# ricklisz/AnatoMask

Hardware: AMD Instinct MI355X
Metric: pretrain volumes/sec @128^3 patch mask=0.6 (higher is better)
Workload: dtype bf16; 1 GPU; STUNet-B AnatoMask step, 128^3 patch, mask_ratio 0.6, bf16 storage/MFMA + fp32 master; per_gpu_batch=16, global_batch=16, parallelism=dp1, step=teacher fwd + sampler + student fwd + loss + bwd + clip + AdamW + EMA

## Files before the change

anatomask_amd/csrc/conv_igemm.hip:

```cpp
#include <mutex>
#include <type_traits>
#include <stdlib.h>
#include "common.h"
#include "../../include/anatomask_hip.h"
#include "conv_plan.h"

using namespace amconv;

namespace {

template <typename T, int BD, int BH, int BW, int NS, int NIT, int TGS = 3, bool HR = false, bool NB = false, bool HT = false>
__global__ __launch_bounds__(256, (TGS == 2 && BD * BH * BW <= 256) ? 3 : 2) void conv_igemm_kernel(ConvArgs a) {
  constexpr int EPC = TT<T>::EPC;
  constexpr bool SPL = std::is_same<T, f32s_t>::value;
  constexpr int KC = (ROWB / 16) * EPC;
  constexpr int MV = BD * BH * BW;
  constexpr int VS = MV / 64;
  constexpr int NT = 16 * NS;
  constexpr int TG = TG_OF(NS, TGS);
  constexpr int WBUF = TG * NT * ROWB;
  constexpr int WCH = TG * NT * 4;
  constexpr int WIT = (WCH + 255) / 256;
  static_assert(MV % 64 == 0, "brick must give each wave whole 16-voxel subtiles");
  extern __shared__ __attribute__((aligned(16))) unsigned char lds[];
// ... 566 lines not shown
#ifdef AM_ABLATE
    { const char* e = getenv("AM_CV_NOLIST"); if (e && atoi(e)) listed = false; }
#endif
    if (listed) {
      a.plist = active_list; a.pbd = qblock / P.bd; a.pbh = qblock / P.bh; a.pbw = qblock / P.bw;
      a.nlive = p.n_active * a.pbd * a.pbh * a.pbw;
    }
  }
  if (p.partials && p.dtype == AM_DT_BF16) {
    const size_t tile = (size_t)P.bd * P.bh * P.bw * (P.nt_tile * 2 + 32);
    if (P.lds < tile) P.lds = tile;
  }
  if (p.nbred) {
    const size_t tiles = (size_t)P.bd * P.bh * P.bw * (P.nt_tile * 4 + 32);
    if (P.lds < tiles) P.lds = tiles;
  }
  a.nt_store = ((size_t)p.B * p.Do * p.Ho * p.Wo * p.Cout * 2 >= ((size_t)384 << 20) && !p.accumulate) || AM_DBG(a, 8);
  hipStream_t st = (hipStream_t)stream;
  if (rows) *rows = (a.plist ? a.nlive : a.B * a.nbd * a.nbh * a.nbw) * a.nclass;
  return p.dtype == AM_DT_BF16 ? dispatch<bf16_t>(P, shape, st) : p.dtype == AM_DT_F32S ? dispatch<f32s_t>(P, shape, st) : dispatch<float>(P, shape, st);
}

#define AM_STAGE_ROW(name_) {#name_, name_##_fits, name_##_serves, name_##_launch}
static const ConvStage conv_stages[] = {AM_STAGE_ROW(conv_k3t), AM_STAGE_ROW(conv_k3), AM_STAGE_ROW(conv_rw), AM_STAGE_ROW(conv_gather), AM_STAGE_ROW(conv_igemm)};

static void query_masks(ConvProblem& p, bool sparse, int in_bshift, int out_bshift, int n_active) {
  p.in_sparse = p.out_sparse = sparse; p.same_mask = p.has_list = true;
  p.in_bshift = in_bshift; p.out_bshift = out_bshift; p.n_active = n_active;
}

extern "C" int am_conv3d_partials_rows(int mode, int dtype, int ksize, int stride, int B, int Do, int Ho, int Wo, int Cin, int Cout, int out_sparse,
                                       int out_bshift, int n_active, int* rows) {
  ConvProblem p{mode, dtype, ksize, stride, B, Do, Ho, Wo, Cin, Do, Ho, Wo, Cout};
  query_masks(p, out_sparse != 0, out_bshift, out_bshift, n_active);
  *rows = 0;
  for (const ConvStage& s : conv_stages) { const int r = s.fits(p); if (r > *rows) *rows = r; }
  return 0;
}

extern "C" int am_conv3d_uses_k3(int mode, int dtype, int ksize, int stride, int B, int Di, int Hi, int Wi, int Cin, int Do, int Ho, int Wo, int Cout,
                                 int has_masks, int accumulate, int fused_epilogue, int want_partials) {
  ConvProblem p{mode, dtype, ksize, stride, B, Di, Hi, Wi, Cin, Do, Ho, Wo, Cout};
  query_masks(p, has_masks != 0, 0, 0, 0);
  p.accumulate = accumulate != 0; p.ep = fused_epilogue != 0; p.partials = want_partials != 0;
  for (const ConvStage& s : conv_stages)
    if (s.serves(p)) return s.launch == conv_k3t_launch ? 2 : s.launch == conv_k3_launch ? 1 : 0;
  return 0;
}

static ConvArgs fill_args(const ConvProblem& p, const void* x, const void* w_packed, const float* bias, void* y, float* partials, const uint8_t* in_mask,
                          int in_bshift, const uint8_t* out_mask, int out_bshift, int fd, int fh, int fw, int accumulate) {
  ConvArgs a{};
  a.x = x; a.w = w_packed; a.bias = bias; a.y = y; a.partials = partials;
  a.B = p.B; a.Di = p.Di; a.Hi = p.Hi; a.Wi = p.Wi; a.Cin = p.Cin; a.Do = p.Do; a.Ho = p.Ho; a.Wo = p.Wo; a.Cout = p.Cout;
  am_packed_dims(p.dtype, p.Cout, p.Cin, &a.Coutp, &a.Cinp);
  a.w_bytes = p.ksize * p.ksize * p.ksize * a.Coutp * a.Cinp * (p.dtype == AM_DT_BF16 ? 2 : 4);
  a.in_mask = MaskView{in_mask, fd, fh, fw, in_bshift};
  a.out_mask = MaskView{out_mask, fd, fh, fw, out_bshift};
  a.accumulate = accumulate & 1; a.stats_sum_only = (accumulate & AM_CONV_PARTIALS_SUM_ONLY) ? 1 : 0;
#ifdef AM_ABLATE
  { const char* e = getenv("AM_CV_DBG"); a.dbg = e ? atoi(e) : 0; }
#endif
  return a;
}

static int conv3d_impl(ConvProblem& p, ConvArgs& a, const int* active_list, int n_active, void* stream, int* rows) {
  if (p.Cin % 8 || p.Cout % 8) return -1;
  p.in_sparse = a.in_mask.m != nullptr; p.out_sparse = a.out_mask.m != nullptr; p.same_mask = a.in_mask.m == a.out_mask.m;
  p.in_bshift = a.in_mask.bs; p.out_bshift = a.out_mask.bs; p.fd = a.in_mask.fd; p.fh = a.in_mask.fh; p.fw = a.in_mask.fw;
  p.has_list = active_list != nullptr; p.n_active = n_active;
// ... 57 lines not shown
```

anatomask_amd/csrc/conv_k3.hip:

```cpp
#include <stdlib.h>
#include "common.h"
#include "../../include/anatomask_hip.h"
#include "conv_plan.h"

using namespace amconv;

namespace {

constexpr int KBD = 8, KBH = 4, KBW = 16;
constexpr int KED = KBD + 2, KEH = KBH + 2, KEW = KBW + 2;
constexpr int KPLANE = KEH * KEW;
constexpr int KNROW = KED * KPLANE;
constexpr int KBRICKB = KNROW * 64;
constexpr int KNPIECE = 68;
constexpr int KWSLOT = 3 * 64 * 64;
constexpr int KLDS_W = 2 * KBRICKB;
constexpr int KLDS_TAB = KLDS_W + 2 * KWSLOT;
constexpr int KLDS = KLDS_TAB + 768;
#ifndef AM_K3_MIN_UNITS
#define AM_K3_MIN_UNITS 256
#endif
constexpr int K3_MIN_UNITS = AM_K3_MIN_UNITS;

struct K3Args {
// ... 5 lines not shown
  int nt_store;
  unsigned w_bytes;
#ifdef AM_ABLATE
  int dbg;
#endif
};

#define K3_LDSP(off) ((__attribute__((address_space(3))) void*)(lds + (off)))

__device__ __forceinline__ int k3_uni(int v) { return __builtin_amdgcn_readfirstlane(v); }
template <typename P> __device__ __forceinline__ P* k3_uni_ptr(P* p) {
  const unsigned long long v = (unsigned long long)p;
  const unsigned lo = (unsigned)__builtin_amdgcn_readfirstlane((int)(unsigned)v), hi = (unsigned)__builtin_amdgcn_readfirstlane((int)(unsigned)(v >> 32));
  return (P*)(((unsigned long long)hi << 32) | lo);
}

struct Item { int u, k, c0, c1, p; };
#define IT_Q0W(it) (((it).c0 & 255) * KBW)
#define IT_Q0H(it) ((((it).c0 >> 8) & 255) * KBH)
#define IT_Q0D(it) ((((it).c0 >> 16) & 255) * KBD)
#define IT_B(it) ((it).c1 & 255)
#define IT_CO0(it) (((it).c1 >> 8) * NT)

template <int NS, bool EP, bool ST, bool CT = false, bool S1 = false>
__global__ __launch_bounds__(512, 2) void conv_k3_kernel(K3Args a) {
  static_assert(NS == 4 || NS == 2, "64- or 32-channel output tiles (NS = 2: the decoder's last conv, C -> C / 2 = 32 at STUNet-B; a wave then owns 8 accumulator tiles)");
  constexpr int VS = 4, NT = 16 * NS;
  constexpr int NCH = VS * NS / 2;
  constexpr int NRUN = CT ? 4 : 9;
  constexpr int NTR = CT ? 2 : 3;
  static_assert(!CT || (NS == 4 && !EP && !ST), "transposed conv: 64-channel tiles, plain epilogue (bias)");
  static_assert(!S1 || (ST && NS == 4 && !CT), "sum-only statistics: a variant of the statistics instantiation");
  extern __shared__ __attribute__((aligned(16))) unsigned char lds[];
  const int tid = threadIdx.x, lane = tid & 63;
  const int wave = __builtin_amdgcn_readfirstlane(tid >> 6);
  const bool isX = wave < 4;
  const int wq = wave & 3;
  const int g = lane >> 4, r16 = lane & 15;
  const int G = gridDim.x;

  const int gperm = (G % 8 == 0) ? (int)(blockIdx.x % 8) * (G / 8) + (int)(blockIdx.x / 8) : (int)blockIdx.x;
  auto decode = [&](Item& it) {
    int br = it.u / a.ny;
    const int yt = it.u - br * a.ny;
    const int bw_ = br % a.nbw; br /= a.nbw;
    const int bh_ = br % a.nbh; br /= a.nbh;
    const int bd_ = br % a.nbd;
    it.c0 = k3_uni(bw_ | (bh_ << 8) | (bd_ << 16)); it.c1 = k3_uni((br / a.nbd) | (yt << 8));
  };
  auto advance = [&](Item& it) {
    if (it.k + 1 < a.nslab) { ++it.k; return; }
    it.k = 0;
    if (CT && it.p < 7) { ++it.p; return; }
    it.p = 0; it.u += G;
    if (it.u < a.nunit) decode(it);
  };
  Item cur; cur.u = gperm; cur.k = 0; cur.p = 0;
  if (cur.u >= a.nunit) return;
  decode(cur);
  Item nxt = cur; advance(nxt);

  const __amdgpu_buffer_rsrc_t rw = __builtin_amdgcn_make_buffer_rsrc((void*)a.w, 0, (int)a.w_bytes, 0x00020000);
  constexpr unsigned OOB = 0x80000000u;
  const int wtapB = a.Coutp * a.Cinp * 2;

  const int wrow = lane >> 2;
  const unsigned wlane = (unsigned)(((((wrow >> 2) & 3) * 8 + (wrow & 3)) * a.Cinp + (((lane & 3) ^ ((wrow >> 1) & 2)) * 8)) * 2);
  const int aoff = swz(r16, g);
  int bx[3];
#pragma unroll
  for (int xw = 0; xw < 3; ++xw) bx[xw] = (wave * KPLANE + r16 + xw) * 64 + ((g ^ (((r16 + xw) >> 2) & 1) * 2) << 4);

  unsigned pl[9], pbits[2] = {0u, 0u};
#pragma unroll
  for (int k = 0; k < 9; ++k) {
    const int p = wave + 8 * k;
    const int row0 = p * 16 < KNROW - 16 ? p * 16 : KNROW - 16;
    const int rho = row0 + (lane >> 2);
    const int z = rho / KPLANE, rem = rho - z * KPLANE, yy = rem / KEW, xx = rem - yy * KEW;
    pl[k] = (unsigned)((((z * a.H + yy) * a.W + xx) * a.Cin + (((lane & 3) ^ (((xx >> 2) & 1) * 2)) * 8)) * 2);
    const unsigned code = (z == 0 ? 1u : 0u) | (z == KED - 1 ? 2u : 0u) | (yy == 0 ? 4u : 0u) | (yy == KEH - 1 ? 8u : 0u) | (xx == 0 ? 16u : 0u) | (xx == KEW - 1 ? 32u : 0u);
    pbits[k / 5] |= code << (6 * (k % 5));
  }

  auto issue_weights = [&](const Item& it, const int run, const int slot) __attribute__((always_inline)) {
    const int pd_ = (it.p >> 2) & 1, ph_ = (it.p >> 1) & 1, pw_ = it.p & 1;
    const int zd = CT ? pd_ + (run >> 1) : run / 3, xw = CT ? pw_ + (run & 1) : run - (run / 3) * 3;
    if (wq >= NS) return;
#pragma unroll
    for (int th = 0; th < NTR; ++th) {
      const int t = zd * 9 + th * 3 + xw;
      const int widx = CT ? ((3 - 2 * zd + pd_) * 4 + (3 - 2 * (ph_ + th) + ph_)) * 4 + (3 - 2 * xw + pw_) : (a.flip ? 26 - t : t);
      const unsigned so = (unsigned)(widx * wtapB + ((IT_CO0(it) + (wq >> 1) * 32 + (wq & 1) * 4) * a.Cinp + it.k * 32) * 2);
#ifdef AM_ABLATE
      if (a.dbg & 4) continue;
#endif
      __builtin_amdgcn_raw_ptr_buffer_load_lds(rw, K3_LDSP(KLDS_W + slot * KWSLOT + th * (NT * 64) + wq * 1024), 16, wlane, so, 0, 0);
    }
  };
  auto issue_pieces = [&](const Item& it, const int sbuf, const int k0, const int k1) __attribute__((always_inline)) {
    const int q0d = IT_Q0D(it), q0h = IT_Q0H(it), q0w = IT_Q0W(it);
    const unsigned m = (q0d == 0 ? 1u : 0u) | (q0d + KBD == a.D ? 2u : 0u) | (q0h == 0 ? 4u : 0u) | (q0h + KBH == a.H ? 8u : 0u) |
                       (q0w == 0 ? 16u : 0u) | (q0w + KBW == a.W ? 32u : 0u);
    const long long org = ((((long long)IT_B(it) * a.D + (q0d - 1)) * a.H + (q0h - 1)) * a.W + (q0w - 1)) * (long long)a.Cin;
    const __amdgpu_buffer_rsrc_t rx = __builtin_amdgcn_make_buffer_rsrc((void*)k3_uni_ptr(a.x + org), 0, 0x7fffff00, 0x00020000);
#pragma unroll
    for (int k = k0; k < k1; ++k) {
      const unsigned bad = pbits[k / 5] & (m << (6 * (k % 5)));
      unsigned vo = bad ? OOB : pl[k];
#ifdef AM_ABLATE
      if (a.dbg & 2) vo = OOB;
#endif
      const int p = wave + 8 * k;
      const int row0 = p * 16 < KNROW - 16 ? p * 16 : KNROW - 16;
      __builtin_amdgcn_raw_ptr_buffer_load_lds(rx, K3_LDSP(sbuf * KBRICKB + row0 * 64), 16, vo, (unsigned)(it.k * 64), 0, 0);
    }
  };

  f32x4 acc[NS][VS];
  float f1[NS / 2][4], f2[NS / 2][4];
#pragma unroll
  for (int h = 0; h < NS / 2; ++h)
#pragma unroll
    for (int r = 0; r < 4; ++r) { f1[h][r] = 0.f; f2[h][r] = 0.f; }
  const unsigned oddm = (lane & 1) ? 0xffffffffu : 0u;
#ifdef AM_ABLATE
  const bool want_stats = ST && a.partials != nullptr && !(a.dbg & 32);
#else
  const bool want_stats = ST && a.partials != nullptr;
#endif
  bf16_t* __restrict__ yg = a.y;
  const float act_slope = a.ep_act == AM_ACT_LRELU ? 0.01f : (a.ep_act == AM_ACT_RELU6 ? 0.f : 1.f);
  const float act_hi = a.ep_act == AM_ACT_RELU6 ? 6.f : __builtin_inff();
  constexpr bool fused = EP;
  typedef __attribute__((ext_vector_type(4))) __bf16 bfx4;
  typedef __attribute__((ext_vector_type(8))) __bf16 bfx8;
  typedef __attribute__((ext_vector_type(8))) float f32x8;

  auto flush_stats = [&](const int co0) __attribute__((always_inline)) {
    float* part = a.partials + ((size_t)blockIdx.x * 8 + wave) * a.Cout * 2;
#define K3_DPP_ADD(V, CTRL) V += __builtin_bit_cast(float, __builtin_amdgcn_update_dpp(0, __builtin_bit_cast(int, V), CTRL, 0xF, 0xF, true))
#pragma unroll
    for (int h = 0; h < NS / 2; ++h)
#pragma unroll
      for (int r = 0; r < 4; ++r) {
        float s1 = f1[h][r], s2 = f2[h][r];
        K3_DPP_ADD(s1, 0x4E); K3_DPP_ADD(s1, 0x124); K3_DPP_ADD(s1, 0x128);
        if constexpr (!S1) { K3_DPP_ADD(s2, 0x4E); K3_DPP_ADD(s2, 0x124); K3_DPP_ADD(s2, 0x128); }
        const int c = co0 + h * 32 + g * 8 + (r16 & 1) * 4 + r;
        if (r16 < 2) { part[c * 2] = s1; part[c * 2 + 1] = s2; }
      }
#undef K3_DPP_ADD
  };

  constexpr bool FULL = NS == 4;
  const bool lo8 = r16 < 8;
  const unsigned olane = FULL ? (unsigned)(((r16 & 7) * (CT ? 2 : 1) * a.Cout + (r16 >> 3) * 32 + g * 8) * 2)
                              : (unsigned)((r16 * (CT ? 2 : 1) * a.Cout + g * 8) * 2);
  const unsigned ohalf = (unsigned)(8 * (CT ? 2 : 1) * a.Cout * 2);
  const unsigned olane_own = (unsigned)((r16 * (CT ? 2 : 1) * a.Cout + g * 8) * 2);
  const unsigned orow = (unsigned)((CT ? 4 : 1) * a.W * a.Cout * 2);
  u32x4 pk[VS][NS / 2];
  long long pk_off = 0;
  auto finish_unit = [&](const int pc0, const int pc1, const int pcls) __attribute__((always_inline)) {
    Item it; it.c0 = pc0; it.c1 = pc1;
    const int co0 = IT_CO0(it);
    if constexpr (CT)
      pk_off = ((((long long)IT_B(it) * (2 * a.D) + (2 * (IT_Q0D(it) + wave) + ((pcls >> 2) & 1))) * (2 * a.H) + (2 * IT_Q0H(it) + ((pcls >> 1) & 1))) * (2 * a.W) +
                (2 * IT_Q0W(it) + (pcls & 1))) * (long long)a.Cout + co0;
    else
    pk_off = ((((long long)IT_B(it) * a.D + (IT_Q0D(it) + wave)) * a.H + IT_Q0H(it)) * a.W + IT_Q0W(it)) * (long long)a.Cout + co0;
    f32x4 bia[NS], esc[NS], esh[NS];
    if (a.bias) {
#pragma unroll
      for (int i = 0; i < NS; ++i) bia[i] = *(const f32x4*)(lds + KLDS_TAB + ((i >> 1) * 32 + g * 8 + (i & 1) * 4) * 4);
// ... 38 lines not shown
      }
    }
  };
  auto stats_half = [&](const int c, const int q) __attribute__((always_inline)) {
    const int j = c / (NS / 2), h = c % (NS / 2);
    const u32x4 wv = pk[j][h];
    const unsigned kw = (wv[2 + q] & oddm) | (wv[q] & ~oddm), gw = (wv[q] & oddm) | (wv[2 + q] & ~oddm);
#pragma unroll
    for (int e = 0; e < 2; ++e) {
      const int r = 2 * q + e;
      const float keep = __uint_as_float(e ? (kw & 0xffff0000u) : (kw << 16)), give = __uint_as_float(e ? (gw & 0xffff0000u) : (gw << 16));
      f1[h][r] += keep;
      f1[h][r] += __builtin_bit_cast(float, __builtin_amdgcn_update_dpp(0, __builtin_bit_cast(int, give), 0xB1, 0xF, 0xF, true));
      if constexpr (!S1) {
        f2[h][r] += keep * keep;
        const float g2 = give * give;
        f2[h][r] += __builtin_bit_cast(float, __builtin_amdgcn_update_dpp(0, __builtin_bit_cast(int, g2), 0xB1, 0xF, 0xF, true));
      }
    }
  };
#ifdef AM_K3_NO_SPREAD_STATS
  constexpr bool spread_stats = false;
#else
  const bool spread_stats = ST && !CT && NCH == 8 && a.nslab >= 2;
#endif
  auto store_chunk = [&](const int c, const bool tail) __attribute__((always_inline)) {
    const int j = c / (NS / 2), h = c % (NS / 2);
    const __amdgpu_buffer_rsrc_t ry = __builtin_amdgcn_make_buffer_rsrc((void*)k3_uni_ptr(yg + pk_off), 0, 0x7fffff00, 0x00020000);
#ifdef AM_ABLATE
    if (!(a.dbg & 1))
#endif
    {
      u32x4 sv = pk[j][h];
      unsigned so_ = (unsigned)(j * orow + h * 64);
      if constexpr (FULL) {
        const u32x4 ot = pk[j][h ^ 1];
        u32x4 rx_;
#pragma unroll
        for (int e = 0; e < 4; ++e) rx_[e] = (unsigned)__builtin_amdgcn_update_dpp(0, (int)ot[e], 0x128, 0xF, 0xF, false);
        const bool own = h == 0 ? lo8 : !lo8;
#pragma unroll
        for (int e = 0; e < 4; ++e) sv[e] = own ? sv[e] : rx_[e];
        so_ = (unsigned)(j * orow) + (h ? ohalf : 0u);
      }
      if (a.nt_store) __builtin_amdgcn_raw_buffer_store_b128(sv, ry, olane, so_, 2);
      else __builtin_amdgcn_raw_buffer_store_b128(sv, ry, olane, so_, 0);
      if (tail || FULL) asm volatile("s_nop 4" : "+v"(sv) :: "memory");
    }
    if (want_stats && (tail || !spread_stats)) { stats_half(c, 0); stats_half(c, 1); }
  };

  if (want_stats && a.ny > 1) {
    float* part = a.partials + ((size_t)blockIdx.x * 8 + wave) * a.Cout * 2;
    for (int c = lane; c < a.Cout * 2; c += 64) part[c] = 0.f;
    asm volatile("s_waitcnt vmcnt(0)" ::: "memory");
  }
  if (tid < NT) {
    const int c = IT_CO0(cur) + tid;
    ((float*)(lds + KLDS_TAB))[tid] = a.bias ? a.bias[c] : 0.f;
    ((float*)(lds + KLDS_TAB))[64 + tid] = a.ep_scale ? a.ep_scale[c] : 1.f;
    ((float*)(lds + KLDS_TAB))[128 + tid] = a.ep_scale ? a.ep_shift[c] : 0.f;
  }
  if (isX) { issue_weights(cur, 0, 0); issue_pieces(cur, 0, 0, 9); }
  else issue_pieces(cur, 0, 0, 8);
  asm volatile("s_waitcnt vmcnt(0) lgkmcnt(0)" ::: "memory");
  __builtin_amdgcn_s_barrier();

#ifdef AM_ABLATE
  unsigned tL = 0, tWL = 0, tM = 0, tWM = 0, tE = 0, t_prev = 0;
  unsigned long long rt0 = 0;
  const bool stamps = (a.dbg & 16) != 0;
#define K3_STAMP(ACC) if (stamps) { unsigned long long t_; asm volatile("s_memtime %0\n\ts_waitcnt lgkmcnt(0)" : "=s"(t_) :: "memory"); ACC += (unsigned)t_ - t_prev; t_prev = (unsigned)t_; }
  if (stamps) { unsigned long long t_; asm volatile("s_memtime %0\n\ts_waitcnt lgkmcnt(0)" : "=s"(t_) :: "memory"); t_prev = (unsigned)t_; asm volatile("s_memrealtime %0\n\ts_waitcnt lgkmcnt(0)" : "=s"(rt0) :: "memory"); }
#else
#define K3_STAMP(ACC)
#endif
  int par = 0, sb = 0;
  int pc0 = 0, pc1 = 0, pcls = 0; bool have_prev = false;
  bool spend = false;
  bool pend_stats = false;
#pragma unroll
  for (int i = 0; i < NS; ++i)
#pragma unroll
    for (int j = 0; j < VS; ++j) acc[i][j] = f32x4{0.f, 0.f, 0.f, 0.f};
  while (true) {
    spend = false;
    if (cur.k == 0 && have_prev) {
      finish_unit(pc0, pc1, pcls);
      spend = true; pend_stats = true;
      K3_STAMP(tE);
    } else if (cur.k >= 2) pend_stats = false;
    const bool has_next = nxt.u < a.nunit;
    int bxc[3];
#pragma unroll
    for (int xw = 0; xw < 3; ++xw) bxc[xw] = bx[xw] + sb * KBRICKB;
    const bool fetch_next = has_next && (!CT || a.nslab != 2 || nxt.p == 0);
    const int cpd = (cur.p >> 2) & 1, cph = (cur.p >> 1) & 1, cpw = cur.p & 1;
#pragma unroll
    for (int run = 0; run < NRUN; ++run) {
      const int zd = run / 3, xw = run % 3;
      u32x4 brow[VS + 2], af[3][NS];
      const int wbase = KLDS_W + par * KWSLOT + aoff;
      if constexpr (CT) {
        const int zq = cpd + (run >> 1), xq = cpw + (run & 1);
        const int bsel = (xq == 0 ? bxc[0] : (xq == 1 ? bxc[1] : bxc[2])) + (zq * KPLANE + cph * KEW) * 64;
#pragma unroll
        for (int r = 0; r < VS + 1; ++r) brow[r] = *(const u32x4*)(lds + bsel + r * KEW * 64);
      } else {
#pragma unroll
      for (int r = 0; r < VS + 2; ++r) brow[r] = *(const u32x4*)(lds + bxc[xw] + (zd * KPLANE + r * KEW) * 64);
      }
#pragma unroll
      for (int th = 0; th < NTR; ++th)
#pragma unroll
        for (int i = 0; i < NS; ++i) af[th][i] = *(const u32x4*)(lds + wbase + th * (NT * 64) + i * 1024);
      const int pk0 = CT ? (isX ? 3 * run : 4 * run) : (run == 0 ? 0 : (run == 1 ? 1 : run + 1));
      const int npx = CT ? (run < 3 ? 3 : 0) : (run == 1 ? 2 : (run < 8 ? 1 : 0));
      const int npy = CT ? (run < 2 ? 4 : 0) : (run == 1 ? 2 : (run < 7 ? 1 : 0));
      constexpr int SPR = CT ? 2 : 1;
      if (isX) {
        if (run < NRUN - 1) issue_weights(cur, run + 1, par ^ 1);
        else if (has_next) issue_weights(nxt, 0, par ^ 1);
        if (fetch_next && npx > 0) issue_pieces(nxt, sb ^ 1, CT ? 3 * run : pk0, (CT ? 3 * run : pk0) + npx);
        if (spend && run * SPR < NCH) {
#pragma unroll
          for (int q = 0; q < SPR; ++q) store_chunk(run * SPR + q, false);
        }
      } else {
        if (spend && run * SPR < NCH) {
#pragma unroll
          for (int q = 0; q < SPR; ++q) store_chunk(run * SPR + q, false);
        }
        if (fetch_next && npy > 0) issue_pieces(nxt, sb ^ 1, CT ? 4 * run : pk0, (CT ? 4 * run : pk0) + npy);
      }
      if (spread_stats && want_stats && pend_stats) {
        if (cur.k == 0) stats_half(run >> 1, run & 1);
        else if (cur.k == 1 && 9 + run < 16) stats_half((9 + run) >> 1, (9 + run) & 1);
      }
      K3_STAMP(tL);
      if (!isX) {
        asm volatile("s_waitcnt lgkmcnt(0)" ::: "memory");
        __builtin_amdgcn_s_barrier();
        K3_STAMP(tWL);
      }
      __builtin_amdgcn_sched_barrier(0);
      __builtin_amdgcn_s_setprio(1);
#ifdef AM_ABLATE
      if (!(a.dbg & 8))
#endif
#pragma unroll
      for (int th = 0; th < NTR; ++th)
#pragma unroll
        for (int j = 0; j < VS; ++j)
#pragma unroll
          for (int i = 0; i < NS; ++i) acc[i][j] = mma_chunk<bf16_t>(af[th][i], brow[j + th], acc[i][j]);
      __builtin_amdgcn_s_setprio(0);
      __builtin_amdgcn_sched_barrier(0);
      if (isX) {
        const int nbehind = (fetch_next ? npx : 0) + ((spend && run * SPR < NCH) ? SPR : 0);
        if (nbehind == 0) asm volatile("s_waitcnt vmcnt(0)" ::: "memory");
        else if (nbehind == 1) asm volatile("s_waitcnt vmcnt(1)" ::: "memory");
        else if (nbehind == 2) asm volatile("s_waitcnt vmcnt(2)" ::: "memory");
        else if (nbehind == 3) asm volatile("s_waitcnt vmcnt(3)" ::: "memory");
        else if (nbehind == 4) asm volatile("s_waitcnt vmcnt(4)" ::: "memory");
        else asm volatile("s_waitcnt vmcnt(5)" ::: "memory");
      } else if (run == NRUN - 2) {
        if (spend && run * SPR < NCH) { if (SPR == 2) asm volatile("s_waitcnt vmcnt(2)" ::: "memory"); else asm volatile("s_waitcnt vmcnt(1)" ::: "memory"); }
        else asm volatile("s_waitcnt vmcnt(0)" ::: "memory");
      }
      K3_STAMP(tM);
      if (isX) {
        __builtin_amdgcn_s_barrier();
        K3_STAMP(tWM);
      }
      par ^= 1;
    }
    sb ^= 1;
    if (cur.k + 1 == a.nslab) { pc0 = cur.c0; pc1 = cur.c1; pcls = cur.p; have_prev = true; }
    if (!has_next) break;
    cur = nxt; advance(nxt);
  }
  finish_unit(pc0, pc1, pcls);
#pragma unroll
  for (int c = 0; c < NCH; ++c) store_chunk(c, true);
  if (want_stats) flush_stats((pc1 >> 8) * NT);
#ifdef AM_ABLATE
  if (stamps && a.partials) {
    K3_STAMP(tE);
    unsigned long long rt1; asm volatile("s_memrealtime %0\n\ts_waitcnt lgkmcnt(0)" : "=s"(rt1) :: "memory");
    unsigned* row = (unsigned*)(a.partials + ((size_t)blockIdx.x * 8 + wave) * a.Cout * 2);
    asm volatile("s_waitcnt vmcnt(0)" ::: "memory");
    if (lane == 0) { row[0] = tL; row[1] = tWL; row[2] = tM; row[3] = tWM; row[4] = tE; row[5] = (unsigned)(rt1 - rt0); }
  }
#endif
}

}

namespace amconv {

static int k3_tiles(int Cout) { return Cout % 64 ? Cout / 32 : Cout / 64; }
// ... 23 lines not shown
#endif
  if (!conv_k3_fits(p) || p.prenorm || p.accumulate || p.nbred) return false;
  if (p.Di != p.Do || p.Hi != p.Ho || p.Wi != p.Wo) return false;
  if ((size_t)(KED + 1) * p.Hi * p.Wi * p.Cin * 2 >= 0x7fffff00ull) return false;
  if (p.ep && p.partials) return false;
  return true;
}

int conv_k3t_fits(const ConvProblem&) { return 0; }
bool conv_k3t_serves(const ConvProblem& p) {
#ifdef AM_ABLATE
  if (getenv("AM_CV_NORW")) return false;
  { const char* e_ = getenv("AM_CV_NOK3T"); if (e_ && atoi(e_)) return false; }
#endif
  if (p.mode != AM_CONVT_FWD || p.dtype != AM_DT_BF16 || p.ksize != 4 || p.stride != 2 || p.in_sparse || p.out_sparse) return false;
  if (p.prenorm || p.accumulate || p.nbred || p.partials || p.ep) return false;
  if (p.Cin % 32 || p.Cin < 64 || p.Cout % 64 || p.Di % KBD || p.Hi % KBH || p.Wi % KBW) return false;
  if (p.Do != 2 * p.Di || p.Ho != 2 * p.Hi || p.Wo != 2 * p.Wi) return false;
  if (p.B > 255 || p.Di / KBD > 255 || p.Hi / KBH > 255 || p.Wi / KBW > 255) return false;
  if ((size_t)(KED + 1) * p.Hi * p.Wi * p.Cin * 2 >= 0x7fffff00ull || (size_t)16 * p.Wo * p.Cout * 2 >= 0x7fffff00ull) return false;
  return k3_units(p.B, p.Di, p.Hi, p.Wi, p.Cout) >= K3_MIN_UNITS;
}

static void k3_fill(K3Args& a, const ConvProblem& p, const ConvArgs& c) {
  a.x = (const bf16_t*)c.x; a.w = (const bf16_t*)c.w; a.bias = c.bias; a.y = (bf16_t*)c.y; a.partials = c.partials;
  a.ep_scale = c.ep_scale; a.ep_shift = c.ep_shift; a.ep_res = (const bf16_t*)c.ep_res; a.ep_act = c.ep_act;
  a.B = c.B; a.D = c.Di; a.H = c.Hi; a.W = c.Wi; a.Cin = c.Cin; a.Cout = c.Cout; a.Cinp = c.Cinp; a.Coutp = c.Coutp;
  a.nbd = c.Di / KBD; a.nbh = c.Hi / KBH; a.nbw = c.Wi / KBW; a.ny = k3_tiles(c.Cout); a.nunit = k3_units(c.B, c.Di, c.Hi, c.Wi, c.Cout); a.nslab = c.Cinp / 32;
  a.flip = p.mode == AM_CONV_DGRAD;
  a.nt_store = (size_t)c.B * c.Do * c.Ho * c.Wo * c.Cout * 2 >= ((size_t)384 << 20);
  a.w_bytes = (unsigned)c.w_bytes;
#ifdef AM_ABLATE
  { const char* e = getenv("AM_K3_DBG"); a.dbg = e ? atoi(e) : 0; }
#endif
}

int conv_k3_launch(const ConvProblem& p, ConvArgs& c, const int*, void* stream, int* rows) {
  if (!conv_k3_serves(p)) return 0;
  const int dev = am_device();
  K3Args a;
  k3_fill(a, p, c);
  const int G = k3_grid(a.nunit, c.Cout, dev);
  auto kern = p.ep ? conv_k3_kernel<4, true, false> : (a.partials ? conv_k3_kernel<4, false, true> : conv_k3_kernel<4, false, false>);
  if (c.Cout % 64) kern = p.ep ? conv_k3_kernel<2, true, false> : (a.partials ? conv_k3_kernel<2, false, true> : conv_k3_kernel<2, false, false>);
  else if (a.partials && !p.ep && c.stats_sum_only) kern = conv_k3_kernel<4, false, true, false, true>;
  AM_HIP_STAGE((am_lds_optin<conv_k3_kernel<4, true, false>, conv_k3_kernel<4, false, true>, conv_k3_kernel<4, false, false>,
                             conv_k3_kernel<2, true, false>, conv_k3_kernel<2, false, true>, conv_k3_kernel<2, false, false>,
                             conv_k3_kernel<4, false, true, false, true>>(dev)));
  AM_LAUNCH(kern, dim3(G), dim3(512), KLDS, (hipStream_t)stream, a);
  AM_CHECK_LAUNCH_STAGE();
  if (rows) *rows = G * 8;
  return 1;
}

int conv_k3t_launch(const ConvProblem& p, ConvArgs& c, const int*, void* stream, int*) {
  if (!conv_k3t_serves(p)) return 0;
  const int dev = am_device();
  K3Args a;
  k3_fill(a, p, c);
  constexpr auto kern = conv_k3_kernel<4, false, false, true>;
  AM_HIP_STAGE(am_lds_optin<kern>(dev));
  AM_LAUNCH(kern, dim3(k3_grid(a.nunit, c.Cout, dev)), dim3(512), KLDS, (hipStream_t)stream, a);
  AM_CHECK_LAUNCH_STAGE();
  return 1;
}

}
```

anatomask_amd/csrc/conv_plan.h:

```cpp
#pragma once
#include "common.h"

namespace amconv {

struct ConvArgs {
  const void* x; const void* w; const float* bias; void* y; float* partials;
  const float* ep_scale; const float* ep_shift; const void* ep_res; int ep_act;
  const void* nb_x; const float* nb_scale; const float* nb_shift; int nb_act;
  const float* in_scale; const float* in_shift; int in_act;
  int B, Di, Hi, Wi, Cin, Do, Ho, Wo, Cout, Cinp, Coutp;
  int OS, GS, nclass, nunit;
  int ny;
  int nbd, nbh, nbw;
  int tap_begin[9];
  int upar[8];
  int taps[64];
  int mind[8], minh[8], minw[8];
  int ed[8], eh[8], ew[8];
  int mdiv_w[8], mdiv_hw[8];
  int w_bytes;
  int w_lds_off;
  MaskView in_mask, out_mask;
  int accumulate;
  int stats_sum_only;
// ... 78 lines not shown
  a.w_lds_off = (int)brick;
  P.tgs = a.nunit > 1 ? 2 : 3;
  P.lds = a.w_lds_off + 2 * TG_OF(P.nt_tile / 16, P.tgs) * P.nt_tile * ROWB;
  return 0;
}


struct ConvProblem {
  int mode, dtype, ksize, stride, B, Di, Hi, Wi, Cin, Do, Ho, Wo, Cout;
  bool in_sparse, out_sparse, same_mask, has_list;
  int in_bshift, out_bshift, n_active, fd, fh, fw;
  bool accumulate, ep, partials, sum_only;
  bool nbred, prenorm;
};

struct ConvStage {
  const char* name;
  int (*fits)(const ConvProblem&);
  bool (*serves)(const ConvProblem&);
  int (*launch)(const ConvProblem&, ConvArgs& a, const int* active_list, void* stream, int* rows);
};
#define AM_CONV_STAGE(name_) int name_##_fits(const ConvProblem&); bool name_##_serves(const ConvProblem&); \
                             int name_##_launch(const ConvProblem&, ConvArgs&, const int*, void*, int*)
AM_CONV_STAGE(conv_k3t); AM_CONV_STAGE(conv_k3);
AM_CONV_STAGE(conv_rw); AM_CONV_STAGE(conv_gather);
AM_CONV_STAGE(conv_igemm);

}
```

anatomask_amd/engine.py:

```python
from __future__ import annotations

from dataclasses import dataclass, field
from typing import Dict, List, Optional, Sequence, Tuple

import torch

from . import ops
from .ops import ACT_LRELU, ACT_NONE, ACT_RELU6, CONV_DGRAD, CONV_FWD, CONVT_DGRAD, CONVT_FWD, MaskInfo, NormStats

ENC = "sparse_encoder.sp_cnn.conv_blocks_context"
DEC = "dense_decoder.dec"


@dataclass
class Spec:
    dims: Sequence[int]
    depth: Sequence[int]
    width: int
    input_size: Tuple[int, int, int]
    in_ch: int = 1
    out_ch: int = 1
    downsample: int = 16
    n_stage: int = 5
    sync_bn: bool = False
# ... 404 lines not shown
        dr = ops.conv3d(CONV_DGRAD, dc2, pk.get(W, f"{q}.conv.3.weight", False, True), None, so, 3, 1)
        _wgrad_into(pk, G, f"{q}.conv.3.weight", CONV_FWD, t["r"], dc2, 3, 1)
        dc1 = _instance_norm_backward(dr, t["c1"], t["st1"], ACT_RELU6)
    elif t.get("head"):
        dc2 = ops.proj_norm_bwd(t["c2"], t["st2"], drec, W["dense_decoder.proj.weight"].view(-1), W[f"{q}.conv.4.weight"],
                                W[f"{q}.conv.4.bias"], G[f"{q}.conv.4.weight"], G[f"{q}.conv.4.bias"],
                                G["dense_decoder.proj.weight"].view(-1), G["dense_decoder.proj.bias"])
    else:
        dc2 = ops.norm_backward(g, None, t["c2"], t["st2"], W[f"{q}.conv.4.weight"], ACT_NONE, None, 0,
                                G[f"{q}.conv.4.weight"], G[f"{q}.conv.4.bias"])
    if not t.get("inorm"):
        so = tuple(t["r"].shape[1:4])
        fuse = ops.FUSED_NORM_BWD_REDUCE and dc2.dtype == torch.bfloat16 and t["st1"].sync_world <= 1 and dc2.shape[-1] >= 128
        dr = ops.conv3d(CONV_DGRAD, dc2, pk.get(W, f"{q}.conv.3.weight", False, True), None, so, 3, 1,
                        norm_bwd=(t["c1"], t["st1"], ACT_RELU6) if fuse else None)
        dr, red1 = dr if fuse else (dr, None)
        _wgrad_into(pk, G, f"{q}.conv.3.weight", CONV_FWD, t["r"], dc2, 3, 1)
        dc1 = ops.norm_backward(dr, None, t["c1"], t["st1"], W[f"{q}.conv.1.weight"], ACT_RELU6, None, 0,
                                G[f"{q}.conv.1.weight"], G[f"{q}.conv.1.bias"], reduced=red1)
    du, ptu = ops.conv3d(CONV_DGRAD, dc1, pk.get(W, f"{q}.conv.0.weight", False, True), None, so, 3, 1, want_partials=True, partials_sum_only=True)
    ptu.finalize(None, sum_accum=G[f"{q}.up_sample.bias"])
    _wgrad_into(pk, G, f"{q}.conv.0.weight", CONV_FWD, t["u"], dc1, 3, 1)
    si = tuple(t["xin"].shape[1:4])
    gin = ops.conv3d(CONVT_DGRAD, du, pk.get(W, f"{q}.up_sample.weight", True, True), None, si, 4, 2, want_partials=bias_sum_into is not None)
    if bias_sum_into is not None:
        gin, ptg = gin
        ptg.finalize(None, sum_accum=bias_sum_into)
    _wgrad_into(pk, G, f"{q}.up_sample.weight", CONVT_FWD, t["xin"], du, 4, 2, transposed=True)
    return gin


def decoder_backward(spec: Spec, W, G, pk: PackCache, tape: Tape, drec: torch.Tensor, after_group=None) -> List[Optional[torch.Tensor]]:
    n_dec = len(spec.dec_chs) - 1
    fused_head = bool(tape.dec[n_dec - 1].get("head"))
    g = None
    if not fused_head:
        g = ops.proj_bwd(tape.last, drec, W["dense_decoder.proj.weight"].view(-1), G["dense_decoder.proj.weight"].view(-1),
                         G["dense_decoder.proj.bias"], deterministic=pk.deterministic)
        if after_group:
            after_group("proj")
    dproj: List[Optional[torch.Tensor]] = [None] * n_dec
    for i in reversed(range(n_dec)):
        t = tape.dec[i]
        if tape.recompute:
            _, t = _dec_block(W, pk, i, t["xin"], t["nxt"], True, update_running=False, sync=spec.sync_bn, head=bool(t.get("head")),
                              inorm=spec.dec_inorm)
            tape.dec[i] = None
# ... 213 lines not shown
```

include/anatomask_hip.h:

```cpp
#ifndef ANATOMASK_HIP_H
#define ANATOMASK_HIP_H
#include <stdint.h>
#ifdef __cplusplus
extern "C" {
#endif

#define AM_DT_F32 0
#define AM_DT_BF16 1
#define AM_DT_F32S 2

#define AM_CONV_PARTIALS_SUM_ONLY 2
#define AM_CONV_FWD 0
#define AM_CONV_DGRAD 1
#define AM_CONVT_FWD 2
#define AM_CONVT_DGRAD 3

#define AM_DXREP 64
#define AM_NREP 8

#define AM_ACT_NONE 0
#define AM_ACT_LRELU 1
#define AM_ACT_RELU6 2

int am_version(void);
// ... 6 lines not shown
              const void* ep_res ,
              int ep_act ,
              const int32_t* active_list, int n_active ,
              int* partial_rows_written ,
              void* stream);
int am_conv3d_prenorm_supported(int mode, int dtype, int ksize, int stride, int B, int Do, int Ho, int Wo, int Cin, int Cout, int sparse,
                                int in_bshift, int out_bshift, int n_active);
int am_conv3d_prenorm(int mode, int dtype, int ksize, int stride, const void* x, const void* w_packed, const float* bias, void* y, int B, int Di,
                      int Hi, int Wi, int Cin, int Do, int Ho, int Wo, int Cout, const uint8_t* mask, int in_bshift, int out_bshift, int fd,
                      int fh, int fw, float* partials , const float* in_scale, const float* in_shift, int in_act,
                      const int32_t* active_list, int n_active, int* partial_rows_written , void* stream);

int am_conv3d_nbred(int mode, int dtype, int ksize, int stride, const void* x, const void* w_packed, void* y, int B, int Di,
                    int Hi, int Wi, int Cin, int Do, int Ho, int Wo, int Cout, const uint8_t* in_mask, int in_bshift,
                    const uint8_t* out_mask, int out_bshift, int fd, int fh, int fw, int accumulate, float* partials,
                    const void* nb_x, const float* nb_scale, const float* nb_shift, int nb_act,
                    int* partial_rows_written, void* stream);
int am_packed_dims(int dtype, int rows, int k, int* rows_padded, int* k_padded);
int am_conv3d_partials_rows(int mode, int dtype, int ksize, int stride, int B, int Do, int Ho, int Wo, int Cin, int Cout,
                            int out_sparse, int out_bshift ,
                            int n_active, int* rows );
int am_conv3d_uses_k3(int mode, int dtype, int ksize, int stride, int B, int Di, int Hi, int Wi, int Cin, int Do, int Ho, int Wo, int Cout,
                      int has_masks, int accumulate, int fused_epilogue, int want_partials);
int am_partials_reduce(const float* partials, int rows, int C, double* sums, float* sum_accum, void* stream);

int am_conv3d_wgrad(int mode, int dtype, int ksize, int stride, const void* x, const void* dy, float* dw_packed,
                    int B, int Dx, int Hx, int Wx, int Cx, int Dy, int Hy, int Wy, int Cy,
                    const uint8_t* x_mask, int x_bshift, const uint8_t* y_mask, int y_bshift, int fd, int fh, int fw,
                    float* det_workspace, long det_workspace_floats,
                    const int32_t* active_list, int n_active ,
                    void* gather_workspace, long gather_workspace_bytes ,
                    void* stream);
int am_conv3d_wgrad_uses_k3(int mode, int dtype, int ksize, int stride, int B, int D, int H, int W, int Cx, int Cy, int has_masks,
                            int deterministic);
int am_conv3d_wgrad_gather_bytes(int mode, int dtype, int ksize, int stride, int B, int Cx, int Cy, int y_bshift, int has_y_mask, int n_active,
                                 int fd, int fh, int fw, long* bytes );

int am_split_bf16(const float* x, void* hi, void* lo, long n, void* stream);

int am_pack_weight(int dtype, const float* src, void* dst, int R, int K, int taps, long stride_r, long stride_k, int Rp, int Kp,
                   void* stream);
typedef struct am_pack_desc {
  const float* src; void* dst; long stride_r, stride_k; int R, K, taps, Rp, Kp, first_block;
} am_pack_desc;
int am_pack_weights_batched(int dtype, const am_pack_desc* descs, int ndesc, int total_blocks, void* stream);
int am_unpack_grad(const float* src_packed, float* dst, int R, int K, int taps, long stride_r, long stride_k, int accumulate,
// ... 173 lines not shown
```

Before: 140.4 volumes/s.

## Route transposed-conv data gradient through the k3 brick kernel with parity phases

Adds a conv_k3td stage that computes the data gradient of the stride-2, 4x4x4 transposed conv on the k3 LDS-brick MFMA kernel. Each output brick iterates the 8 input parity phases as 2x2x2-tap runs over a stride-2 view of the input, accumulating all phases before the epilogue. Per-block channel statistics are reduced across waves in LDS, and the decoder requests sum-only partials. This replaces the generic igemm/gather path for these decoder backward convs, at the cost of more kernel variants and new indexing that could be wrong at edges.

```diff
diff --git a/anatomask_amd/csrc/conv_igemm.hip b/anatomask_amd/csrc/conv_igemm.hip
--- a/anatomask_amd/csrc/conv_igemm.hip
+++ b/anatomask_amd/csrc/conv_igemm.hip
@@ -1,5 +1,6 @@
 #include <mutex>
 #include <type_traits>
+#include <stdio.h>
 #include <stdlib.h>
 #include "common.h"
 #include "../../include/anatomask_hip.h"
@@ -612,7 +613,7 @@
 }
 
 #define AM_STAGE_ROW(name_) {#name_, name_##_fits, name_##_serves, name_##_launch}
-static const ConvStage conv_stages[] = {AM_STAGE_ROW(conv_k3t), AM_STAGE_ROW(conv_k3), AM_STAGE_ROW(conv_rw), AM_STAGE_ROW(conv_gather), AM_STAGE_ROW(conv_igemm)};
+static const ConvStage conv_stages[] = {AM_STAGE_ROW(conv_k3t), AM_STAGE_ROW(conv_k3td), AM_STAGE_ROW(conv_k3), AM_STAGE_ROW(conv_rw), AM_STAGE_ROW(conv_gather), AM_STAGE_ROW(conv_igemm)};
 
 static void query_masks(ConvProblem& p, bool sparse, int in_bshift, int out_bshift, int n_active) {
   p.in_sparse = p.out_sparse = sparse; p.same_mask = p.has_list = true;
@@ -636,6 +637,17 @@
   for (const ConvStage& s : conv_stages)
     if (s.serves(p)) return s.launch == conv_k3t_launch ? 2 : s.launch == conv_k3_launch ? 1 : 0;
   return 0;
+}
+
+extern "C" int am_conv3d_stage_name(int mode, int dtype, int ksize, int stride, int B, int Di, int Hi, int Wi, int Cin, int Do, int Ho, int Wo, int Cout,
+                                    int has_masks, int accumulate, int fused_epilogue, int want_partials, char* name, int cap) {
+  if (!name || cap <= 0) return -1;
+  ConvProblem p{mode, dtype, ksize, stride, B, Di, Hi, Wi, Cin, Do, Ho, Wo, Cout};
+  query_masks(p, has_masks != 0, 0, 0, 0);
+  p.accumulate = accumulate != 0; p.ep = fused_epilogue != 0; p.partials = want_partials != 0;
+  for (const ConvStage& s : conv_stages)
+    if (s.serves(p)) { snprintf(name, (size_t)cap, "%s", s.name); return 0; }
+  return -7;
 }
 
 static ConvArgs fill_args(const ConvProblem& p, const void* x, const void* w_packed, const float* bias, void* y, float* partials, const uint8_t* in_mask,
diff --git a/anatomask_amd/csrc/conv_k3.hip b/anatomask_amd/csrc/conv_k3.hip
--- a/anatomask_amd/csrc/conv_k3.hip
+++ b/anatomask_amd/csrc/conv_k3.hip
@@ -51,15 +51,17 @@
 #define IT_B(it) ((it).c1 & 255)
 #define IT_CO0(it) (((it).c1 >> 8) * NT)
 
-template <int NS, bool EP, bool ST, bool CT = false, bool S1 = false>
+template <int NS, bool EP, bool ST, bool CT = false, bool S1 = false, bool CD = false>
 __global__ __launch_bounds__(512, 2) void conv_k3_kernel(K3Args a) {
   static_assert(NS == 4 || NS == 2, "64- or 32-channel output tiles (NS = 2: the decoder's last conv, C -> C / 2 = 32 at STUNet-B; a wave then owns 8 accumulator tiles)");
   constexpr int VS = 4, NT = 16 * NS;
   constexpr int NCH = VS * NS / 2;
-  constexpr int NRUN = CT ? 4 : 9;
-  constexpr int NTR = CT ? 2 : 3;
+  constexpr bool C2 = CT || CD;
+  constexpr int NRUN = C2 ? 4 : 9;
+  constexpr int NTR = C2 ? 2 : 3;
   static_assert(!CT || (NS == 4 && !EP && !ST), "transposed conv: 64-channel tiles, plain epilogue (bias)");
   static_assert(!S1 || (ST && NS == 4 && !CT), "sum-only statistics: a variant of the statistics instantiation");
+  static_assert(!CD || (NS == 4 && !EP && !CT), "transposed conv's data gradient: 64-channel tiles, no fused store epilogue");
   extern __shared__ __attribute__((aligned(16))) unsigned char lds[];
   const int tid = threadIdx.x, lane = tid & 63;
   const int wave = __builtin_amdgcn_readfirstlane(tid >> 6);
@@ -80,7 +82,7 @@
   auto advance = [&](Item& it) {
     if (it.k + 1 < a.nslab) { ++it.k; return; }
     it.k = 0;
-    if (CT && it.p < 7) { ++it.p; return; }
+    if (C2 && it.p < 7) { ++it.p; return; }
     it.p = 0; it.u += G;
     if (it.u < a.nunit) decode(it);
   };
@@ -107,19 +109,21 @@
     const int row0 = p * 16 < KNROW - 16 ? p * 16 : KNROW - 16;
     const int rho = row0 + (lane >> 2);
     const int z = rho / KPLANE, rem = rho - z * KPLANE, yy = rem / KEW, xx = rem - yy * KEW;
-    pl[k] = (unsigned)((((z * a.H + yy) * a.W + xx) * a.Cin + (((lane & 3) ^ (((xx >> 2) & 1) * 2)) * 8)) * 2);
+    pl[k] = CD ? (unsigned)((((z * 4 * a.H + yy * 2) * 2 * a.W + xx * 2) * a.Cin + (((lane & 3) ^ (((xx >> 2) & 1) * 2)) * 8)) * 2)
+               : (unsigned)((((z * a.H + yy) * a.W + xx) * a.Cin + (((lane & 3) ^ (((xx >> 2) & 1) * 2)) * 8)) * 2);
     const unsigned code = (z == 0 ? 1u : 0u) | (z == KED - 1 ? 2u : 0u) | (yy == 0 ? 4u : 0u) | (yy == KEH - 1 ? 8u : 0u) | (xx == 0 ? 16u : 0u) | (xx == KEW - 1 ? 32u : 0u);
     pbits[k / 5] |= code << (6 * (k % 5));
   }
 
   auto issue_weights = [&](const Item& it, const int run, const int slot) __attribute__((always_inline)) {
     const int pd_ = (it.p >> 2) & 1, ph_ = (it.p >> 1) & 1, pw_ = it.p & 1;
-    const int zd = CT ? pd_ + (run >> 1) : run / 3, xw = CT ? pw_ + (run & 1) : run - (run / 3) * 3;
+    const int zd = C2 ? pd_ + (run >> 1) : run / 3, xw = C2 ? pw_ + (run & 1) : run - (run / 3) * 3;
     if (wq >= NS) return;
 #pragma unroll
     for (int th = 0; th < NTR; ++th) {
       const int t = zd * 9 + th * 3 + xw;
-      const int widx = CT ? ((3 - 2 * zd + pd_) * 4 + (3 - 2 * (ph_ + th) + ph_)) * 4 + (3 - 2 * xw + pw_) : (a.flip ? 26 - t : t);
+      const int wct = ((3 - 2 * zd + pd_) * 4 + (3 - 2 * (ph_ + th) + ph_)) * 4 + (3 - 2 * xw + pw_);
+      const int widx = CT ? wct : (CD ? 63 - wct : (a.flip ? 26 - t : t));
       const unsigned so = (unsigned)(widx * wtapB + ((IT_CO0(it) + (wq >> 1) * 32 + (wq & 1) * 4) * a.Cinp + it.k * 32) * 2);
 #ifdef AM_ABLATE
       if (a.dbg & 4) continue;
@@ -131,7 +135,9 @@
     const int q0d = IT_Q0D(it), q0h = IT_Q0H(it), q0w = IT_Q0W(it);
     const unsigned m = (q0d == 0 ? 1u : 0u) | (q0d + KBD == a.D ? 2u : 0u) | (q0h == 0 ? 4u : 0u) | (q0h + KBH == a.H ? 8u : 0u) |
                        (q0w == 0 ? 16u : 0u) | (q0w + KBW == a.W ? 32u : 0u);
-    const long long org = ((((long long)IT_B(it) * a.D + (q0d - 1)) * a.H + (q0h - 1)) * a.W + (q0w - 1)) * (long long)a.Cin;
+    const long long org = CD ? ((((long long)IT_B(it) * (2 * a.D) + (2 * (q0d - 1) + 1 - ((it.p >> 2) & 1))) * (2 * a.H) + (2 * (q0h - 1) + 1 - ((it.p >> 1) & 1))) * (2 * a.W) +
+                                (2 * (q0w - 1) + 1 - (it.p & 1))) * (long long)a.Cin
+                             : ((((long long)IT_B(it) * a.D + (q0d - 1)) * a.H + (q0h - 1)) * a.W + (q0w - 1)) * (long long)a.Cin;
     const __amdgpu_buffer_rsrc_t rx = __builtin_amdgcn_make_buffer_rsrc((void*)k3_uni_ptr(a.x + org), 0, 0x7fffff00, 0x00020000);
 #pragma unroll
     for (int k = k0; k < k1; ++k) {
@@ -167,7 +173,9 @@
   typedef __attribute__((ext_vector_type(8))) float f32x8;
 
   auto flush_stats = [&](const int co0) __attribute__((always_inline)) {
-    float* part = a.partials + ((size_t)blockIdx.x * 8 + wave) * a.Cout * 2;
+    float* part = a.partials + (CD ? (size_t)blockIdx.x : (size_t)blockIdx.x * 8 + wave) * a.Cout * 2;
+    float* sc = (float*)lds;
+    if constexpr (CD) __syncthreads();
 #define K3_DPP_ADD(V, CTRL) V += __builtin_bit_cast(float, __builtin_amdgcn_update_dpp(0, __builtin_bit_cast(int, V), CTRL, 0xF, 0xF, true))
 #pragma unroll
     for (int h = 0; h < NS / 2; ++h)
@@ -177,9 +185,19 @@
         K3_DPP_ADD(s1, 0x4E); K3_DPP_ADD(s1, 0x124); K3_DPP_ADD(s1, 0x128);
         if constexpr (!S1) { K3_DPP_ADD(s2, 0x4E); K3_DPP_ADD(s2, 0x124); K3_DPP_ADD(s2, 0x128); }
         const int c = co0 + h * 32 + g * 8 + (r16 & 1) * 4 + r;
-        if (r16 < 2) { part[c * 2] = s1; part[c * 2 + 1] = s2; }
+        if constexpr (CD) { if (r16 < 2) { sc[(wave * 64 + (c - co0)) * 2] = s1; sc[(wave * 64 + (c - co0)) * 2 + 1] = s2; } }
+        else if (r16 < 2) { part[c * 2] = s1; part[c * 2 + 1] = s2; }
       }
 #undef K3_DPP_ADD
+    if constexpr (CD) {
+      __syncthreads();
+      if (wave == 0) {
+        float t1 = 0.f, t2 = 0.f;
+#pragma unroll
+        for (int w = 0; w < 8; ++w) { t1 += sc[(w * 64 + lane) * 2]; t2 += sc[(w * 64 + lane) * 2 + 1]; }
+        part[(co0 + lane) * 2] = t1; part[(co0 + lane) * 2 + 1] = t2;
+      }
+    }
   };
 
   constexpr bool FULL = NS == 4;
@@ -264,7 +282,7 @@
 #ifdef AM_K3_NO_SPREAD_STATS
   constexpr bool spread_stats = false;
 #else
-  const bool spread_stats = ST && !CT && NCH == 8 && a.nslab >= 2;
+  const bool spread_stats = ST && !C2 && NCH == 8 && a.nslab >= 2;
 #endif
   auto store_chunk = [&](const int c, const bool tail) __attribute__((always_inline)) {
     const int j = c / (NS / 2), h = c % (NS / 2);
@@ -292,8 +310,8 @@
     if (want_stats && (tail || !spread_stats)) { stats_half(c, 0); stats_half(c, 1); }
   };
 
-  if (want_stats && a.ny > 1) {
-    float* part = a.partials + ((size_t)blockIdx.x * 8 + wave) * a.Cout * 2;
+  if (want_stats && a.ny > 1 && (!CD || wave == 0)) {
+    float* part = a.partials + (CD ? (size_t)blockIdx.x : (size_t)blockIdx.x * 8 + wave) * a.Cout * 2;
     for (int c = lane; c < a.Cout * 2; c += 64) part[c] = 0.f;
     asm volatile("s_waitcnt vmcnt(0)" ::: "memory");
   }
@@ -327,7 +345,7 @@
     for (int j = 0; j < VS; ++j) acc[i][j] = f32x4{0.f, 0.f, 0.f, 0.f};
   while (true) {
     spend = false;
-    if (cur.k == 0 && have_prev) {
+    if (cur.k == 0 && have_prev && (!CD || cur.p == 0)) {
       finish_unit(pc0, pc1, pcls);
       spend = true; pend_stats = true;
       K3_STAMP(tE);
@@ -343,7 +361,7 @@
       const int zd = run / 3, xw = run % 3;
       u32x4 brow[VS + 2], af[3][NS];
       const int wbase = KLDS_W + par * KWSLOT + aoff;
-      if constexpr (CT) {
+      if constexpr (C2) {
         const int zq = cpd + (run >> 1), xq = cpw + (run & 1);
         const int bsel = (xq == 0 ? bxc[0] : (xq == 1 ? bxc[1] : bxc[2])) + (zq * KPLANE + cph * KEW) * 64;
 #pragma unroll
@@ -356,14 +374,14 @@
       for (int th = 0; th < NTR; ++th)
 #pragma unroll
         for (int i = 0; i < NS; ++i) af[th][i] = *(const u32x4*)(lds + wbase + th * (NT * 64) + i * 1024);
-      const int pk0 = CT ? (isX ? 3 * run : 4 * run) : (run == 0 ? 0 : (run == 1 ? 1 : run + 1));
-      const int npx = CT ? (run < 3 ? 3 : 0) : (run == 1 ? 2 : (run < 8 ? 1 : 0));
-      const int npy = CT ? (run < 2 ? 4 : 0) : (run == 1 ? 2 : (run < 7 ? 1 : 0));
-      constexpr int SPR = CT ? 2 : 1;
+      const int pk0 = C2 ? (isX ? 3 * run : 4 * run) : (run == 0 ? 0 : (run == 1 ? 1 : run + 1));
+      const int npx = C2 ? (run < 3 ? 3 : 0) : (run == 1 ? 2 : (run < 8 ? 1 : 0));
+      const int npy = C2 ? (run < 2 ? 4 : 0) : (run == 1 ? 2 : (run < 7 ? 1 : 0));
+      constexpr int SPR = C2 ? 2 : 1;
       if (isX) {
         if (run < NRUN - 1) issue_weights(cur, run + 1, par ^ 1);
         else if (has_next) issue_weights(nxt, 0, par ^ 1);
-        if (fetch_next && npx > 0) issue_pieces(nxt, sb ^ 1, CT ? 3 * run : pk0, (CT ? 3 * run : pk0) + npx);
+        if (fetch_next && npx > 0) issue_pieces(nxt, sb ^ 1, C2 ? 3 * run : pk0, (C2 ? 3 * run : pk0) + npx);
         if (spend && run * SPR < NCH) {
 #pragma unroll
           for (int q = 0; q < SPR; ++q) store_chunk(run * SPR + q, false);
@@ -373,7 +391,7 @@
 #pragma unroll
           for (int q = 0; q < SPR; ++q) store_chunk(run * SPR + q, false);
         }
-        if (fetch_next && npy > 0) issue_pieces(nxt, sb ^ 1, CT ? 4 * run : pk0, (CT ? 4 * run : pk0) + npy);
+        if (fetch_next && npy > 0) issue_pieces(nxt, sb ^ 1, C2 ? 4 * run : pk0, (C2 ? 4 * run : pk0) + npy);
       }
       if (spread_stats && want_stats && pend_stats) {
         if (cur.k == 0) stats_half(run >> 1, run & 1);
@@ -418,7 +436,7 @@
       par ^= 1;
     }
     sb ^= 1;
-    if (cur.k + 1 == a.nslab) { pc0 = cur.c0; pc1 = cur.c1; pcls = cur.p; have_prev = true; }
+    if (cur.k + 1 == a.nslab && (!CD || cur.p == 7)) { pc0 = cur.c0; pc1 = cur.c1; pcls = cur.p; have_prev = true; }
     if (!has_next) break;
     cur = nxt; advance(nxt);
   }
@@ -488,11 +506,36 @@
   return k3_units(p.B, p.Di, p.Hi, p.Wi, p.Cout) >= K3_MIN_UNITS;
 }
 
+static int k3td_rows(const ConvProblem& p) { return k3_grid(k3_units(p.B, p.Do, p.Ho, p.Wo, p.Cout), p.Cout); }
+static bool k3td_shape(const ConvProblem& p) {
+  if (p.mode != AM_CONVT_DGRAD || p.dtype != AM_DT_BF16 || p.ksize != 4 || p.stride != 2 || p.in_sparse || p.out_sparse) return false;
+  if (p.Cin % 32 || p.Cin < 64 || p.Cout % 64 || p.Do % KBD || p.Ho % KBH || p.Wo % KBW) return false;
+  if (p.B > 255 || p.Do / KBD > 255 || p.Ho / KBH > 255 || p.Wo / KBW > 255) return false;
+  return k3_units(p.B, p.Do, p.Ho, p.Wo, p.Cout) >= K3_MIN_UNITS;
+}
+int conv_k3td_fits(const ConvProblem& p) {
+  if (!k3td_shape(p)) return 0;
+  const int r = k3td_rows(p);
+  return r <= conv_igemm_fits(p) ? r : 0;
+}
+bool conv_k3td_serves(const ConvProblem& p) {
+#ifdef AM_ABLATE
+  if (getenv("AM_CV_NORW")) return false;
+  { const char* e_ = getenv("AM_CV_NOK3TD"); if (e_ && atoi(e_)) return false; }
+#endif
+  if (!k3td_shape(p) || p.prenorm || p.accumulate || p.nbred || p.ep) return false;
+  if (p.Di != 2 * p.Do || p.Hi != 2 * p.Ho || p.Wi != 2 * p.Wo) return false;
+  if (p.partials && !conv_k3td_fits(p)) return false;
+  if ((size_t)2 * (KED + 1) * p.Hi * p.Wi * p.Cin * 2 >= 0x7fffff00ull) return false;
+  return true;
+}
+
 static void k3_fill(K3Args& a, const ConvProblem& p, const ConvArgs& c) {
   a.x = (const bf16_t*)c.x; a.w = (const bf16_t*)c.w; a.bias = c.bias; a.y = (bf16_t*)c.y; a.partials = c.partials;
   a.ep_scale = c.ep_scale; a.ep_shift = c.ep_shift; a.ep_res = (const bf16_t*)c.ep_res; a.ep_act = c.ep_act;
   a.B = c.B; a.D = c.Di; a.H = c.Hi; a.W = c.Wi; a.Cin = c.Cin; a.Cout = c.Cout; a.Cinp = c.Cinp; a.Coutp = c.Coutp;
-  a.nbd = c.Di / KBD; a.nbh = c.Hi / KBH; a.nbw = c.Wi / KBW; a.ny = k3_tiles(c.Cout); a.nunit = k3_units(c.B, c.Di, c.Hi, c.Wi, c.Cout); a.nslab = c.Cinp / 32;
+  if (p.mode == AM_CONVT_DGRAD) { a.D = c.Do; a.H = c.Ho; a.W = c.Wo; }
+  a.nbd = a.D / KBD; a.nbh = a.H / KBH; a.nbw = a.W / KBW; a.ny = k3_tiles(c.Cout); a.nunit = k3_units(c.B, a.D, a.H, a.W, c.Cout); a.nslab = c.Cinp / 32;
   a.flip = p.mode == AM_CONV_DGRAD;
   a.nt_store = (size_t)c.B * c.Do * c.Ho * c.Wo * c.Cout * 2 >= ((size_t)384 << 20);
   a.w_bytes = (unsigned)c.w_bytes;
@@ -531,4 +574,19 @@
   return 1;
 }
 
-}
+int conv_k3td_launch(const ConvProblem& p, ConvArgs& c, const int*, void* stream, int* rows) {
+  if (!conv_k3td_serves(p)) return 0;
+  const int dev = am_device();
+  K3Args a;
+  k3_fill(a, p, c);
+  const int G = k3_grid(a.nunit, c.Cout, dev);
+  constexpr auto plain = conv_k3_kernel<4, false, false, false, false, true>, stat = conv_k3_kernel<4, false, true, false, false, true>,
+                 sum1 = conv_k3_kernel<4, false, true, false, true, true>;
+  AM_HIP_STAGE((am_lds_optin<plain, stat, sum1>(dev)));
+  AM_LAUNCH(a.partials ? (c.stats_sum_only ? sum1 : stat) : plain, dim3(G), dim3(512), KLDS, (hipStream_t)stream, a);
+  AM_CHECK_LAUNCH_STAGE();
+  if (rows) *rows = G;
+  return 1;
+}
+
+}
diff --git a/anatomask_amd/csrc/conv_plan.h b/anatomask_amd/csrc/conv_plan.h
--- a/anatomask_amd/csrc/conv_plan.h
+++ b/anatomask_amd/csrc/conv_plan.h
@@ -124,7 +124,7 @@
 };
 #define AM_CONV_STAGE(name_) int name_##_fits(const ConvProblem&); bool name_##_serves(const ConvProblem&); \
                              int name_##_launch(const ConvProblem&, ConvArgs&, const int*, void*, int*)
-AM_CONV_STAGE(conv_k3t); AM_CONV_STAGE(conv_k3);
+AM_CONV_STAGE(conv_k3t); AM_CONV_STAGE(conv_k3td); AM_CONV_STAGE(conv_k3);
 AM_CONV_STAGE(conv_rw); AM_CONV_STAGE(conv_gather);
 AM_CONV_STAGE(conv_igemm);
 
diff --git a/anatomask_amd/engine.py b/anatomask_amd/engine.py
--- a/anatomask_amd/engine.py
+++ b/anatomask_amd/engine.py
@@ -450,7 +450,8 @@
     ptu.finalize(None, sum_accum=G[f"{q}.up_sample.bias"])
     _wgrad_into(pk, G, f"{q}.conv.0.weight", CONV_FWD, t["u"], dc1, 3, 1)
     si = tuple(t["xin"].shape[1:4])
-    gin = ops.conv3d(CONVT_DGRAD, du, pk.get(W, f"{q}.up_sample.weight", True, True), None, si, 4, 2, want_partials=bias_sum_into is not None)
+    gin = ops.conv3d(CONVT_DGRAD, du, pk.get(W, f"{q}.up_sample.weight", True, True), None, si, 4, 2, want_partials=bias_sum_into is not None,
+                     partials_sum_only=True)
     if bias_sum_into is not None:
         gin, ptg = gin
         ptg.finalize(None, sum_accum=bias_sum_into)
diff --git a/include/anatomask_hip.h b/include/anatomask_hip.h
--- a/include/anatomask_hip.h
+++ b/include/anatomask_hip.h
@@ -52,6 +52,8 @@
                             int n_active, int* rows );
 int am_conv3d_uses_k3(int mode, int dtype, int ksize, int stride, int B, int Di, int Hi, int Wi, int Cin, int Do, int Ho, int Wo, int Cout,
                       int has_masks, int accumulate, int fused_epilogue, int want_partials);
+int am_conv3d_stage_name(int mode, int dtype, int ksize, int stride, int B, int Di, int Hi, int Wi, int Cin, int Do, int Ho, int Wo, int Cout,
+                         int has_masks, int accumulate, int fused_epilogue, int want_partials, char* name, int cap);
 int am_partials_reduce(const float* partials, int rows, int C, double* sums, float* sum_accum, void* stream);
 
 int am_conv3d_wgrad(int mode, int dtype, int ksize, int stride, const void* x, const void* dy, float* dw_packed,
```

Result: no change. 140.2 volumes/s (median of 2 runs) (-0.1%).
